# NVIDIA/semantic-segmentation

Hardware: AMD Instinct MI355X
Metric: train images/sec HRNet-OCR-MScale 1024x1024 crop (higher is better)
Workload: dtype fp16; 1 GPU; train_cityscapes_sota: HRNet-OCR-MScale two-scale train step, RMI+BCE loss, crop 1024x1024, batch 1/GPU, SGD, synthetic Cityscapes-shaped batch, random init; global_batch=1, parallelism=dp1, hipgraph=True, optimizer=ssa_sgd_momentum_step, wgrad_side_stream_flush_at=256

## Files before the change

### semantic-segmentation_amd/csrc/conv_wgrad_head.hip

```cpp
#include "common.h"
#include "group.h"
#include "../../include/semseg_hip.h"

namespace {

typedef short s16x8_t __attribute__((ext_vector_type(8)));

__host__ __device__ constexpr int trs(int row_bytes) {
  int s = (row_bytes + 63) / 64;
  if ((s & 1) == 0) ++s;
  return s * 64;
}

__device__ __forceinline__ bf16x8_t tr8(const unsigned char* p, int stride_bytes) {
  const s16x4_t lo = ssa_tr16_b64(p);
  const s16x4_t hi = ssa_tr16_b64(p + 4 * stride_bytes);
  s16x8_t v = {lo[0], lo[1], lo[2], lo[3], hi[0], hi[1], hi[2], hi[3]};
  return __builtin_bit_cast(bf16x8_t, v);
}

struct WgradHeadArgs {
  const bf16_t* x; const bf16_t* dy; float* partial;
  int ldx, Cin, lddy, cout_pad, B, H, W, tiles_x, tiles_y, tiles_per_wg, ci_tiles, G, wgs_y;
};

__device__ __forceinline__ int xcd_order(int v, int n) {
  const int q = n >> 3, r = n & 7, x = v & 7, k = v >> 3;
  return (x < r ? x * (q + 1) : r * (q + 1) + (x - r) * q) + k;
}

template <int KS>
struct ConvWgradHead {
  typedef WgradHeadArgs Args;
  static constexpr int NT = 512;
  static __device__ __forceinline__ void run(const Args& a, const int bx_, const int by0_, const int ) {
  const int w_ = xcd_order(by0_ * a.G + bx_, a.G * a.wgs_y);
  const int bx = w_ / a.wgs_y, by_ = w_ - bx * a.wgs_y;
  const bf16_t* __restrict__ x = a.x;
  const bf16_t* __restrict__ dy = a.dy;
  float* __restrict__ partial = a.partial;
  const int ldx = a.ldx, Cin = a.Cin, lddy = a.lddy, cout_pad = a.cout_pad, B = a.B, H = a.H, W = a.W;
  const int tiles_x = a.tiles_x, tiles_y = a.tiles_y, tiles_per_wg = a.tiles_per_wg, ci_tiles = a.ci_tiles;
  constexpr int TW = 32, TH = 4, NT = KS == 3 ? 3 : 2;
  constexpr int CX = KS == 3 ? 128 : 256;
  constexpr int XW = KS == 3 ? TW + 2 : TW;
  constexpr int SX = trs(CX * 2), SD = trs(256);
  constexpr int X_BYTES = TH * XW * SX;
  constexpr int XP = CX / 8, DP = 16;
  constexpr int XN = TH * XW * XP, DN = TH * TW * DP;
  constexpr int XI = (XN + 511) / 512, DI = (DN + 511) / 512;
  SSA_DYN_LDS(unsigned char, smem);
  unsigned char* Xs = smem;
  unsigned char* Ds = smem + X_BYTES;

  const int tid = threadIdx.x, lane = tid & 63;
  const int wave = __builtin_amdgcn_readfirstlane(tid >> 6);
  const int wm = wave >> 2, wn = wave & 3;
  int by = by_;
  const int kh = KS == 3 ? by % 3 : 0;
  if (KS == 3) by /= 3;
  const int ci_t = by % ci_tiles, co_t = by / ci_tiles;
  const int co0 = co_t * 128, ci0 = ci_t * CX;
  const int taps = KS * KS, Kflat = taps * Cin;

  const int li = lane & 15, lj = li >> 2, lq = li & 3, lg = (lane >> 4) & 1, lh = lane >> 5;
  int b_off[NT];
#pragma unroll
  for (int j = 0; j < NT; ++j) {
    const int cblk = KS == 3 ? wn : 2 * wn + j;
    const int shift = KS == 3 ? j : 0;
    b_off[j] = shift * SX + (cblk * 32 + 16 * lg + 4 * lq) * 2;
  }
  const int a_col = (16 * lg + 4 * lq) * 2;

  f32x16_t acc[2][NT];
#pragma unroll
  for (int m = 0; m < 2; ++m)
#pragma unroll
    for (int j = 0; j < NT; ++j)
#pragma unroll
      for (int r = 0; r < 16; ++r) acc[m][j][r] = 0.f;

  const int total_tiles = B * tiles_x * tiles_y;
  const int t_begin = bx * tiles_per_wg;
  const int t_end = min(total_tiles, t_begin + tiles_per_wg);
  uint4 xv[XI], dv[DI];
  unsigned xmask = 0, dmask = 0;
  auto fetch = [&](int t) {
    int r_ = t;
    const int tx_i = r_ % tiles_x; r_ /= tiles_x;
    const int ty_i = r_ % tiles_y;
    const int b = r_ / tiles_y;
    const int x0 = tx_i * TW, y0 = ty_i * TH;
    const int yoff = KS == 3 ? kh - 1 : 0, xoff = KS == 3 ? -1 : 0;
    const bf16_t* xb = x + (long)b * H * W * ldx + ci0;
    const bf16_t* db = dy + (long)b * H * W * lddy + co0;
#pragma unroll
    for (int i = 0; i < XI; ++i) {
      const int piece = tid + i * 512;
      const int pix = piece / XP, cp = piece - pix * XP;
      const int hy = pix / XW, hx = pix - hy * XW;
      const int iy = y0 + hy + yoff, ix = x0 + hx + xoff;
      const bool ok = piece < XN && (unsigned)iy < (unsigned)H && (unsigned)ix < (unsigned)W && ci0 + cp * 8 < Cin;
      xv[i] = *reinterpret_cast<const uint4*>(ok ? xb + ((long)iy * W + ix) * ldx + cp * 8 : x);
      xmask = i == 0 ? (ok ? 1u : 0u) : (xmask | ((ok ? 1u : 0u) << i));
    }
#pragma unroll
    for (int i = 0; i < DI; ++i) {
      const int piece = tid + i * 512;
      const int pix = piece / DP, cp = piece - pix * DP;
      const int oy = y0 + pix / TW, ox = x0 + pix % TW;
      const bool ok = piece < DN && oy < H && ox < W && co0 + cp * 8 < cout_pad;
      dv[i] = *reinterpret_cast<const uint4*>(ok ? db + ((long)oy * W + ox) * lddy + cp * 8 : dy);
      dmask = i == 0 ? (ok ? 1u : 0u) : (dmask | ((ok ? 1u : 0u) << i));
    }
  };
  auto stage = [&]() {
#pragma unroll
    for (int i = 0; i < XI; ++i) {
      const int piece = tid + i * 512;
      if (piece < XN)
        *reinterpret_cast<uint4*>(Xs + (piece / XP) * SX + (piece % XP) * 16) = ((xmask >> i) & 1u) ? xv[i] : make_uint4(0, 0, 0, 0);
    }
#pragma unroll
    for (int i = 0; i < DI; ++i) {
      const int piece = tid + i * 512;
      if (piece < DN)
        *reinterpret_cast<uint4*>(Ds + (piece / DP) * SD + (piece % DP) * 16) = ((dmask >> i) & 1u) ? dv[i] : make_uint4(0, 0, 0, 0);
    }
  };

  if (t_begin < t_end) fetch(t_begin);
  for (int t = t_begin; t < t_end; ++t) {
    if (t > t_begin) __syncthreads();
    stage();
    __syncthreads();
    if (t + 1 < t_end) fetch(t + 1);
    bf16x8_t af[2][2], bfr[2][NT];
    auto rd = [&](int ks, int slot) {
      const int ty = ks >> 1, kp = (ks & 1) * 16 + 8 * lh + lj;
#pragma unroll
      for (int m = 0; m < 2; ++m) af[slot][m] = tr8(Ds + (ty * TW + kp) * SD + (wm * 2 + m) * 64 + a_col, SD);
#pragma unroll
      for (int j = 0; j < NT; ++j) bfr[slot][j] = tr8(Xs + (ty * XW + kp) * SX + b_off[j], SX);
    };
    rd(0, 0);
    __builtin_amdgcn_sched_group_barrier(0x100, 2 * (2 + NT), 0);
#pragma unroll
    for (int ks = 0; ks < 8; ++ks) {
      if (ks + 1 < 8) rd(ks + 1, (ks + 1) & 1);
#pragma unroll
      for (int m = 0; m < 2; ++m)
#pragma unroll
        for (int j = 0; j < NT; ++j)
          acc[m][j] = ssa_mfma32(af[ks & 1][m], bfr[ks & 1][j], acc[m][j]);
      if (ks + 1 < 8) __builtin_amdgcn_sched_group_barrier(0x100, 2 * (2 + NT), 0);
      __builtin_amdgcn_sched_group_barrier(0x008, 2 * NT, 0);
    }
  }

  float* out = partial + (long)bx * cout_pad * Kflat;
#pragma unroll
  for (int m = 0; m < 2; ++m)
#pragma unroll
    for (int j = 0; j < NT; ++j) {
      const int cblk = KS == 3 ? wn : 2 * wn + j;
      const int ci = ci0 + cblk * 32 + (lane & 31);
      const int tap = KS == 3 ? kh * 3 + j : 0;
      if (ci >= Cin) continue;
      const long kcol = (long)tap * Cin + ci;
#pragma unroll
      for (int r = 0; r < 16; ++r) {
        const int co = co0 + (wm * 2 + m) * 32 + (r & 3) + 8 * (r >> 2) + 4 * (lane >> 5);
        if (co < cout_pad) out[(long)co * Kflat + kcol] = acc[m][j][r];
      }
    }
  }
};

__device__ uint4 g_zero_piece;

struct ConvWgradHead3 {
  typedef WgradHeadArgs Args;
  static constexpr int NT = 512;
  static constexpr int TW = 32, TH = 4, XW = TW + 2, CX = 128;
  static constexpr int X_BYTES = TH * XW * 256, D_BYTES = TH * TW * 256, BUF_BYTES = X_BYTES + D_BYTES;
  static constexpr int XWI = X_BYTES / 1024;
  static constexpr int XI = (XWI + 7) / 8, DI = D_BYTES / 1024 / 8, NI = XI + DI;
  static_assert(NI == 9, "one DMA in front of the k loop and one behind each of its 8 steps");
  static constexpr size_t LDS = 2 * (size_t)BUF_BYTES + 1024;
  static __device__ __forceinline__ void run(const Args& a, const int bx_, const int by0_, const int ) {
  const int w_ = xcd_order(by0_ * a.G + bx_, a.G * a.wgs_y);
  const int bx = w_ / a.wgs_y;
  int by = w_ - bx * a.wgs_y;
  const bf16_t* __restrict__ x = a.x;
  const bf16_t* __restrict__ dy = a.dy;
  float* __restrict__ partial = a.partial;
  const int ldx = a.ldx, Cin = a.Cin, lddy = a.lddy, cout_pad = a.cout_pad, B = a.B, H = a.H, W = a.W;
  const int tiles_x = a.tiles_x, tiles_y = a.tiles_y, tiles_per_wg = a.tiles_per_wg, ci_tiles = a.ci_tiles;
  SSA_DYN_LDS(unsigned char, smem);
  unsigned char* dump = smem + 2 * BUF_BYTES;

  const int tid = threadIdx.x, lane = tid & 63;
  const int wave = __builtin_amdgcn_readfirstlane(tid >> 6);
  const int wm = wave >> 2, wn = wave & 3;
  const int kh = by % 3; by /= 3;
  const int ci_t = by % ci_tiles, co_t = by / ci_tiles;
  const int co0 = co_t * 128, ci0 = ci_t * CX;
  const int Kflat = 9 * Cin;

  int rel[NI], yx[NI];
#pragma unroll
  for (int i = 0; i < NI; ++i) {
    const bool isx = i < XI;
    const int wi = (isx ? i : i - XI) * 8 + wave;
    const int piece = wi * 64 + lane;
    const int p = piece >> 4, q = (piece & 15) ^ ((p & 3) << 2);
    const int r = isx ? p / XW : p >> 5, c = isx ? p - r * XW : p & 31;
    const bool real = isx ? (wi < XWI && ci0 + q * 8 < Cin) : (co0 + q * 8 < cout_pad);
    rel[i] = (r * W + c) * (isx ? ldx : lddy) + q * 8;
    yx[i] = real ? ((r << 8) | c) : 0xffff;
  }
  int f_tx, f_ty, f_b;
  const int total_tiles = B * tiles_x * tiles_y;
  const int t_begin = bx * tiles_per_wg;
  const int t_end = min(total_tiles, t_begin + tiles_per_wg);
  {
    f_tx = t_begin % tiles_x;
    const int r_ = t_begin / tiles_x;
    f_ty = r_ % tiles_y;
    f_b = r_ / tiles_y;
  }
  const bf16_t* zero_src = reinterpret_cast<const bf16_t*>(&g_zero_piece);
#ifndef SSA_EMU
  asm volatile("" : "+v"(zero_src));
#endif
  auto dma = [&](int i, int buf) {
    const int x0 = f_tx * TW, y0 = f_ty * TH;
    const bool isx = i < XI;
    const int wi = (isx ? i : i - XI) * 8 + wave;
    const int oy = isx ? y0 + kh - 1 : y0, ox = isx ? x0 - 1 : x0;
    const bf16_t* base = (isx ? x + ci0 : dy + co0) + ((long)f_b * H * W + (long)oy * W + ox) * (isx ? ldx : lddy);
    const int iy = oy + (yx[i] >> 8), ix = ox + (yx[i] & 255);
    const bool ok = yx[i] != 0xffff && (unsigned)iy < (unsigned)H && (unsigned)ix < (unsigned)W;
    const bf16_t* src = ok ? base + rel[i] : zero_src;
    unsigned char* Xb = smem + buf * BUF_BYTES;
    unsigned char* dst = isx ? (wi < XWI ? Xb + wi * 1024 : dump) : Xb + X_BYTES + wi * 1024;
    ssa_glds16_untracked(src, dst);
  };
  auto next_tile = [&]() {
    if (++f_tx == tiles_x) {
      f_tx = 0;
      if (++f_ty == tiles_y) { f_ty = 0; ++f_b; }
    }
  };

  const int li = lane & 15, lj = li >> 2, lq = li & 3, lg = (lane >> 4) & 1, lh = lane >> 5;
  const int lrow = (8 * lh + lj) * 256 + lg * 32 + lq * 8;
  int a_base[2], b_base[4];
#pragma unroll
  for (int m = 0; m < 2; ++m) a_base[m] = X_BYTES + lrow + (((wm * 2 + m) ^ lj) << 6);
#pragma unroll
  for (int r = 0; r < 4; ++r) b_base[r] = lrow + ((wn ^ ((lj + r) & 3)) << 6);

  f32x16_t acc[2][3];
#pragma unroll
  for (int m = 0; m < 2; ++m)
#pragma unroll
    for (int j = 0; j < 3; ++j)
#pragma unroll
      for (int r = 0; r < 16; ++r) acc[m][j][r] = 0.f;

  if (t_begin < t_end) {
#pragma unroll
    for (int i = 0; i < NI; ++i) dma(i, 0);
    next_tile();
    ssa_wait_vm_barrier<0, 0>();
  }
  for (int t = t_begin; t < t_end; ++t) {
    const int buf = (t - t_begin) & 1;
    const bool more = t + 1 < t_end;
    if (more) dma(0, buf ^ 1);
    const unsigned char* Tb = smem + buf * BUF_BYTES;
    bf16x8_t af[2][2], bfr[2][3];
    auto rd = [&](int ks, int slot) {
      const int ty = ks >> 1, kp = (ks & 1) * 16;
#pragma unroll
      for (int m = 0; m < 2; ++m) af[slot][m] = tr8(Tb + a_base[m] + (ty * TW + kp) * 256, 256);
#pragma unroll
      for (int j = 0; j < 3; ++j) bfr[slot][j] = tr8(Tb + b_base[(2 * ty + j) & 3] + (ty * XW + kp + j) * 256, 256);
    };
    rd(0, 0);
    __builtin_amdgcn_sched_group_barrier(0x100, 10, 0);
#pragma unroll
    for (int ks = 0; ks < 8; ++ks) {
      if (ks + 1 < 8) rd(ks + 1, (ks + 1) & 1);
#pragma unroll
      for (int m = 0; m < 2; ++m)
#pragma unroll
        for (int j = 0; j < 3; ++j)
          acc[m][j] = ssa_mfma32(af[ks & 1][m], bfr[ks & 1][j], acc[m][j]);
      if (more) dma(ks + 1, buf ^ 1);
      if (ks + 1 < 8) __builtin_amdgcn_sched_group_barrier(0x100, 10, 0);
      __builtin_amdgcn_sched_group_barrier(0x008, 6, 0);
      __builtin_amdgcn_sched_group_barrier(0x020, 1, 0);
    }
    if (more) next_tile();
    ssa_wait_vm_barrier<0, 0>();
  }

  float* out = partial + (long)bx * cout_pad * Kflat;
#pragma unroll
  for (int m = 0; m < 2; ++m)
#pragma unroll
    for (int j = 0; j < 3; ++j) {
      const int ci = ci0 + wn * 32 + (lane & 31);
      if (ci >= Cin) continue;
      const long kcol = (long)(kh * 3 + j) * Cin + ci;
#pragma unroll
      for (int r = 0; r < 16; ++r) {
        const int co = co0 + (wm * 2 + m) * 32 + (r & 3) + 8 * (r >> 2) + 4 * (lane >> 5);
        if (co < cout_pad) out[(long)co * Kflat + kcol] = acc[m][j][r];
      }
    }
  }
};

bool head_shape_ok(const ssa_conv_desc* d, int cout_pad) {
  if (!d || d->KH != d->KW || (d->KH != 3 && d->KH != 1)) return false;
  if (d->stride != 1 || d->dil != 1 || d->pad != d->KH / 2 || d->transposed) return false;
  if (d->Ho != d->H || d->Wo != d->W || d->ldx % 8 || d->Cin % 8 || cout_pad % 8) return false;
  return d->Cin >= 128 && cout_pad >= 64 && d->W >= 32 && (long)d->B * d->H * d->W >= 16384;
}

struct HeadPlan { int co_tiles, ci_tiles, wgs_y, G, tpw; long per_split; };

HeadPlan head_plan(const ssa_conv_desc& d, int cout_pad) {
  HeadPlan p;
  const int cx = d.KH == 3 ? 128 : 256;
  p.co_tiles = (cout_pad + 127) / 128;
  p.ci_tiles = (d.Cin + cx - 1) / cx;
  p.wgs_y = p.co_tiles * p.ci_tiles * (d.KH == 3 ? 3 : 1);
  const long tiles = (long)d.B * ((d.W + 31) / 32) * ((d.H + 3) / 4);
  long g = 256 / p.wgs_y;
  if (g < 1) g = 1;
  if (g > tiles) g = tiles;
  p.tpw = (int)((tiles + g - 1) / g);
  p.G = (int)((tiles + p.tpw - 1) / p.tpw);
  p.per_split = (long)cout_pad * d.KH * d.KW * d.Cin * sizeof(float);
  return p;
}

void fill_args(WgradHeadArgs& a, const ssa_conv_desc& d, const HeadPlan& p, const void* x, const void* dy, int lddy,
               int cout_pad, float* partial) {
  a.x = (const bf16_t*)x; a.dy = (const bf16_t*)dy; a.partial = partial;
  a.ldx = d.ldx; a.Cin = d.Cin; a.lddy = lddy; a.cout_pad = cout_pad; a.B = d.B; a.H = d.H; a.W = d.W;
  a.tiles_x = (d.W + 31) / 32; a.tiles_y = (d.H + 3) / 4; a.tiles_per_wg = p.tpw; a.ci_tiles = p.ci_tiles;
  a.G = p.G; a.wgs_y = p.wgs_y;
}

template <int KS>
int launch_head(const ssa_conv_desc& d, const HeadPlan& p, const void* x, const void* dy, int lddy,
                int cout_pad, float* partial, hipStream_t s) {
  constexpr int XW = KS == 3 ? 34 : 32, CX = KS == 3 ? 128 : 256;
  constexpr size_t lds = (size_t)4 * XW * trs(CX * 2) + (size_t)128 * trs(256);
  static_assert(lds <= 160 * 1024, "does not fit in LDS");
  WgradHeadArgs a;
  fill_args(a, d, p, x, dy, lddy, cout_pad, partial);
  return ssa::submit<ConvWgradHead<KS>>(a, p.G, p.wgs_y, lds, s);
}

}

extern "C" {

int ssa_conv2d_wgrad_head_plan(const ssa_conv_desc* d, int cout_pad, int* nsplit, size_t* ws_bytes) {
  if (!nsplit || !ws_bytes || !head_shape_ok(d, cout_pad)) return SSA_EUNSUPPORTED;
  const HeadPlan p = head_plan(*d, cout_pad);
  *nsplit = p.G;
  *ws_bytes = (size_t)p.G * p.per_split;
  return SSA_OK;
}

int ssa_conv2d_wgrad_head(const ssa_conv_desc* dp, const void* x, const void* dy, int lddy, int cout_pad,
                          int nsplit, float* partial, void* stream) {
  if (!dp || !x || !dy || !partial) return SSA_EINVAL;
  if (!head_shape_ok(dp, cout_pad) || lddy % 8) return SSA_EUNSUPPORTED;
  if ((reinterpret_cast<uintptr_t>(x) | reinterpret_cast<uintptr_t>(dy)) & 15u) return SSA_EINVAL;
  const HeadPlan p = head_plan(*dp, cout_pad);
  if (nsplit != p.G) return SSA_EINVAL;
  if (dp->KH == 3) {
    WgradHeadArgs a;
    fill_args(a, *dp, p, x, dy, lddy, cout_pad, partial);
    return ssa::submit<ConvWgradHead3>(a, p.G, p.wgs_y, ConvWgradHead3::LDS, (hipStream_t)stream);
  }
  return launch_head<1>(*dp, p, x, dy, lddy, cout_pad, partial, (hipStream_t)stream);
}

}
```

Before: 52.37 images/s.

## Restructure head wgrad kernels: async DMA 1x1 path, all-tap 3x3 tiles

The 1x1 head weight-gradient kernel now treats pixels as a flat 64-pixel K dimension. Operands are loaded with double-buffered global-to-LDS DMA and XOR-swizzled LDS, replacing register staging. A selectable 256-wide co tile (MB=8) is chosen by a byte-traffic heuristic, trading fewer passes over x against larger split partials. The 3x3 kernel no longer splits work across kh into separate workgroups: each workgroup loads a 6-row halo with 64 input channels and computes all 9 taps, split 5/4 across two wave groups, which cuts redundant dy reads but raises per-workgroup accumulator pressure.

```diff
diff --git a/semantic-segmentation_amd/csrc/conv_wgrad_head.hip b/semantic-segmentation_amd/csrc/conv_wgrad_head.hip
--- a/semantic-segmentation_amd/csrc/conv_wgrad_head.hip
+++ b/semantic-segmentation_amd/csrc/conv_wgrad_head.hip
@@ -1,16 +1,11 @@
 #include "common.h"
 #include "group.h"
 #include "../../include/semseg_hip.h"
+#include <type_traits>
 
 namespace {
 
 typedef short s16x8_t __attribute__((ext_vector_type(8)));
-
-__host__ __device__ constexpr int trs(int row_bytes) {
-  int s = (row_bytes + 63) / 64;
-  if ((s & 1) == 0) ++s;
-  return s * 64;
-}
 
 __device__ __forceinline__ bf16x8_t tr8(const unsigned char* p, int stride_bytes) {
   const s16x4_t lo = ssa_tr16_b64(p);
@@ -29,170 +24,151 @@
   return (x < r ? x * (q + 1) : r * (q + 1) + (x - r) * q) + k;
 }
 
-template <int KS>
+__device__ uint4 g_zero_piece;
+
+__device__ __forceinline__ const bf16_t* zero_piece() {
+  const bf16_t* z = reinterpret_cast<const bf16_t*>(&g_zero_piece);
+#ifndef SSA_EMU
+  asm volatile("" : "+v"(z));
+#endif
+  return z;
+}
+
+template <int MB>
 struct ConvWgradHead {
   typedef WgradHeadArgs Args;
   static constexpr int NT = 512;
+  static constexpr int KP = 64, CX = 256;
+  static constexpr int SXP = CX * 2, SDP = MB * 64;
+  static constexpr int X_BYTES = KP * SXP, D_BYTES = KP * SDP, BUF_BYTES = X_BYTES + D_BYTES;
+  static constexpr int XI = X_BYTES / 1024 / 8, DI = D_BYTES / 1024 / 8, NI = XI + DI;
+  static constexpr int WM = MB / 2, WN = 8 / WM, NB = 8 / WN;
+  static constexpr size_t LDS = 2 * (size_t)BUF_BYTES;
+  static_assert((MB == 4 || MB == 8) && LDS <= 160 * 1024, "geometry");
   static __device__ __forceinline__ void run(const Args& a, const int bx_, const int by0_, const int ) {
   const int w_ = xcd_order(by0_ * a.G + bx_, a.G * a.wgs_y);
-  const int bx = w_ / a.wgs_y, by_ = w_ - bx * a.wgs_y;
+  const int bx = w_ / a.wgs_y, by = w_ - bx * a.wgs_y;
   const bf16_t* __restrict__ x = a.x;
   const bf16_t* __restrict__ dy = a.dy;
   float* __restrict__ partial = a.partial;
-  const int ldx = a.ldx, Cin = a.Cin, lddy = a.lddy, cout_pad = a.cout_pad, B = a.B, H = a.H, W = a.W;
-  const int tiles_x = a.tiles_x, tiles_y = a.tiles_y, tiles_per_wg = a.tiles_per_wg, ci_tiles = a.ci_tiles;
-  constexpr int TW = 32, TH = 4, NT = KS == 3 ? 3 : 2;
-  constexpr int CX = KS == 3 ? 128 : 256;
-  constexpr int XW = KS == 3 ? TW + 2 : TW;
-  constexpr int SX = trs(CX * 2), SD = trs(256);
-  constexpr int X_BYTES = TH * XW * SX;
-  constexpr int XP = CX / 8, DP = 16;
-  constexpr int XN = TH * XW * XP, DN = TH * TW * DP;
-  constexpr int XI = (XN + 511) / 512, DI = (DN + 511) / 512;
+  const int ldx = a.ldx, Cin = a.Cin, lddy = a.lddy, cout_pad = a.cout_pad;
   SSA_DYN_LDS(unsigned char, smem);
-  unsigned char* Xs = smem;
-  unsigned char* Ds = smem + X_BYTES;
 
   const int tid = threadIdx.x, lane = tid & 63;
   const int wave = __builtin_amdgcn_readfirstlane(tid >> 6);
-  const int wm = wave >> 2, wn = wave & 3;
-  int by = by_;
-  const int kh = KS == 3 ? by % 3 : 0;
-  if (KS == 3) by /= 3;
-  const int ci_t = by % ci_tiles, co_t = by / ci_tiles;
-  const int co0 = co_t * 128, ci0 = ci_t * CX;
-  const int taps = KS * KS, Kflat = taps * Cin;
+  const int wm = wave / WN, wn = wave % WN;
+  const int ci_t = by % a.ci_tiles, co_t = by / a.ci_tiles;
+  const int co0 = co_t * (MB * 32), ci0 = ci_t * CX;
+  const int Kflat = Cin;
+
+  int pk[NI];
+#pragma unroll
+  for (int i = 0; i < NI; ++i) {
+    const bool isx = i < XI;
+    const int slot = ((isx ? i : i - XI) * 8 + wave) * 64 + lane;
+    const int pp = isx ? SXP / 16 : SDP / 16;
+    const int p = slot / pp, q = (slot % pp) ^ ((p & 3) << 2);
+    const bool real = isx ? ci0 + q * 8 < Cin : co0 + q * 8 < cout_pad;
+    pk[i] = real ? ((p << 8) | q) : -1;
+  }
+  const int pixels = a.B * a.H * a.W;
+  const int total = (pixels + KP - 1) / KP;
+  const int s_begin = bx * a.tiles_per_wg;
+  const int s_end = min(total, s_begin + a.tiles_per_wg);
+  const bf16_t* zero_src = zero_piece();
+  auto dma = [&](int i, int s, int buf) {
+    const bool isx = i < XI;
+    const int wi = (isx ? i : i - XI) * 8 + wave;
+    const int pix = s * KP + (pk[i] >> 8);
+    const bool ok = pk[i] >= 0 && pix < pixels;
+    const bf16_t* src = ok ? (isx ? x + ci0 + (long)pix * ldx : dy + co0 + (long)pix * lddy) + (pk[i] & 255) * 8 : zero_src;
+    ssa_glds16_untracked(src, smem + buf * BUF_BYTES + (isx ? 0 : X_BYTES) + wi * 1024);
+  };
 
   const int li = lane & 15, lj = li >> 2, lq = li & 3, lg = (lane >> 4) & 1, lh = lane >> 5;
-  int b_off[NT];
-#pragma unroll
-  for (int j = 0; j < NT; ++j) {
-    const int cblk = KS == 3 ? wn : 2 * wn + j;
-    const int shift = KS == 3 ? j : 0;
-    b_off[j] = shift * SX + (cblk * 32 + 16 * lg + 4 * lq) * 2;
-  }
-  const int a_col = (16 * lg + 4 * lq) * 2;
-
-  f32x16_t acc[2][NT];
+  const int lcol = lg * 32 + lq * 8;
+  int a_base[2], b_base[NB];
+#pragma unroll
+  for (int m = 0; m < 2; ++m) a_base[m] = X_BYTES + (8 * lh + lj) * SDP + lcol + (((wm * 2 + m) ^ lj) << 6);
+#pragma unroll
+  for (int j = 0; j < NB; ++j) b_base[j] = (8 * lh + lj) * SXP + lcol + (((wn * NB + j) ^ lj) << 6);
+
+  f32x16_t acc[2][NB];
 #pragma unroll
   for (int m = 0; m < 2; ++m)
 #pragma unroll
-    for (int j = 0; j < NT; ++j)
+    for (int j = 0; j < NB; ++j)
 #pragma unroll
       for (int r = 0; r < 16; ++r) acc[m][j][r] = 0.f;
 
-  const int total_tiles = B * tiles_x * tiles_y;
-  const int t_begin = bx * tiles_per_wg;
-  const int t_end = min(total_tiles, t_begin + tiles_per_wg);
-  uint4 xv[XI], dv[DI];
-  unsigned xmask = 0, dmask = 0;
-  auto fetch = [&](int t) {
-    int r_ = t;
-    const int tx_i = r_ % tiles_x; r_ /= tiles_x;
-    const int ty_i = r_ % tiles_y;
-    const int b = r_ / tiles_y;
-    const int x0 = tx_i * TW, y0 = ty_i * TH;
-    const int yoff = KS == 3 ? kh - 1 : 0, xoff = KS == 3 ? -1 : 0;
-    const bf16_t* xb = x + (long)b * H * W * ldx + ci0;
-    const bf16_t* db = dy + (long)b * H * W * lddy + co0;
-#pragma unroll
-    for (int i = 0; i < XI; ++i) {
-      const int piece = tid + i * 512;
-      const int pix = piece / XP, cp = piece - pix * XP;
-      const int hy = pix / XW, hx = pix - hy * XW;
-      const int iy = y0 + hy + yoff, ix = x0 + hx + xoff;
-      const bool ok = piece < XN && (unsigned)iy < (unsigned)H && (unsigned)ix < (unsigned)W && ci0 + cp * 8 < Cin;
-      xv[i] = *reinterpret_cast<const uint4*>(ok ? xb + ((long)iy * W + ix) * ldx + cp * 8 : x);
-      xmask = i == 0 ? (ok ? 1u : 0u) : (xmask | ((ok ? 1u : 0u) << i));
-    }
-#pragma unroll
-    for (int i = 0; i < DI; ++i) {
-      const int piece = tid + i * 512;
-      const int pix = piece / DP, cp = piece - pix * DP;
-      const int oy = y0 + pix / TW, ox = x0 + pix % TW;
-      const bool ok = piece < DN && oy < H && ox < W && co0 + cp * 8 < cout_pad;
-      dv[i] = *reinterpret_cast<const uint4*>(ok ? db + ((long)oy * W + ox) * lddy + cp * 8 : dy);
-      dmask = i == 0 ? (ok ? 1u : 0u) : (dmask | ((ok ? 1u : 0u) << i));
-    }
-  };
-  auto stage = [&]() {
-#pragma unroll
-    for (int i = 0; i < XI; ++i) {
-      const int piece = tid + i * 512;
-      if (piece < XN)
-        *reinterpret_cast<uint4*>(Xs + (piece / XP) * SX + (piece % XP) * 16) = ((xmask >> i) & 1u) ? xv[i] : make_uint4(0, 0, 0, 0);
-    }
-#pragma unroll
-    for (int i = 0; i < DI; ++i) {
-      const int piece = tid + i * 512;
-      if (piece < DN)
-        *reinterpret_cast<uint4*>(Ds + (piece / DP) * SD + (piece % DP) * 16) = ((dmask >> i) & 1u) ? dv[i] : make_uint4(0, 0, 0, 0);
-    }
-  };
-
-  if (t_begin < t_end) fetch(t_begin);
-  for (int t = t_begin; t < t_end; ++t) {
-    if (t > t_begin) __syncthreads();
-    stage();
-    __syncthreads();
-    if (t + 1 < t_end) fetch(t + 1);
-    bf16x8_t af[2][2], bfr[2][NT];
+  if (s_begin < s_end) {
+#pragma unroll
+    for (int i = 0; i < NI; ++i) dma(i, s_begin, 0);
+    ssa_wait_vm_barrier<0, 0>();
+  }
+  for (int s = s_begin; s < s_end; ++s) {
+    const int buf = (s - s_begin) & 1;
+    const bool more = s + 1 < s_end;
+    const unsigned char* Tb = smem + buf * BUF_BYTES;
+    bf16x8_t af[2][2], bfr[2][NB];
     auto rd = [&](int ks, int slot) {
-      const int ty = ks >> 1, kp = (ks & 1) * 16 + 8 * lh + lj;
-#pragma unroll
-      for (int m = 0; m < 2; ++m) af[slot][m] = tr8(Ds + (ty * TW + kp) * SD + (wm * 2 + m) * 64 + a_col, SD);
-#pragma unroll
-      for (int j = 0; j < NT; ++j) bfr[slot][j] = tr8(Xs + (ty * XW + kp) * SX + b_off[j], SX);
+#pragma unroll
+      for (int m = 0; m < 2; ++m) af[slot][m] = tr8(Tb + a_base[m] + ks * 16 * SDP, SDP);
+#pragma unroll
+      for (int j = 0; j < NB; ++j) bfr[slot][j] = tr8(Tb + b_base[j] + ks * 16 * SXP, SXP);
     };
     rd(0, 0);
-    __builtin_amdgcn_sched_group_barrier(0x100, 2 * (2 + NT), 0);
-#pragma unroll
-    for (int ks = 0; ks < 8; ++ks) {
-      if (ks + 1 < 8) rd(ks + 1, (ks + 1) & 1);
+    __builtin_amdgcn_sched_group_barrier(0x100, 2 * (2 + NB), 0);
+#pragma unroll
+    for (int ks = 0; ks < 4; ++ks) {
+      if (ks + 1 < 4) rd(ks + 1, (ks + 1) & 1);
 #pragma unroll
       for (int m = 0; m < 2; ++m)
 #pragma unroll
-        for (int j = 0; j < NT; ++j)
+        for (int j = 0; j < NB; ++j)
           acc[m][j] = ssa_mfma32(af[ks & 1][m], bfr[ks & 1][j], acc[m][j]);
-      if (ks + 1 < 8) __builtin_amdgcn_sched_group_barrier(0x100, 2 * (2 + NT), 0);
-      __builtin_amdgcn_sched_group_barrier(0x008, 2 * NT, 0);
-    }
+      if (more) {
+#pragma unroll
+        for (int i = ks * NI / 4; i < (ks + 1) * NI / 4; ++i) dma(i, s + 1, buf ^ 1);
+      }
+      if (ks + 1 < 4) __builtin_amdgcn_sched_group_barrier(0x100, 2 * (2 + NB), 0);
+      __builtin_amdgcn_sched_group_barrier(0x008, 2 * NB, 0);
+      __builtin_amdgcn_sched_group_barrier(0x020, (NI + 3) / 4, 0);
+    }
+    ssa_wait_vm_barrier<0, 0>();
   }
 
   float* out = partial + (long)bx * cout_pad * Kflat;
 #pragma unroll
   for (int m = 0; m < 2; ++m)
 #pragma unroll
-    for (int j = 0; j < NT; ++j) {
-      const int cblk = KS == 3 ? wn : 2 * wn + j;
-      const int ci = ci0 + cblk * 32 + (lane & 31);
-      const int tap = KS == 3 ? kh * 3 + j : 0;
+    for (int j = 0; j < NB; ++j) {
+      const int ci = ci0 + (wn * NB + j) * 32 + (lane & 31);
       if (ci >= Cin) continue;
-      const long kcol = (long)tap * Cin + ci;
 #pragma unroll
       for (int r = 0; r < 16; ++r) {
         const int co = co0 + (wm * 2 + m) * 32 + (r & 3) + 8 * (r >> 2) + 4 * (lane >> 5);
-        if (co < cout_pad) out[(long)co * Kflat + kcol] = acc[m][j][r];
+        if (co < cout_pad) out[(long)co * Kflat + ci] = acc[m][j][r];
       }
     }
   }
 };
-
-__device__ uint4 g_zero_piece;
 
 struct ConvWgradHead3 {
   typedef WgradHeadArgs Args;
   static constexpr int NT = 512;
-  static constexpr int TW = 32, TH = 4, XW = TW + 2, CX = 128;
-  static constexpr int X_BYTES = TH * XW * 256, D_BYTES = TH * TW * 256, BUF_BYTES = X_BYTES + D_BYTES;
-  static constexpr int XWI = X_BYTES / 1024;
+  static constexpr int TW = 32, TH = 4, XW = TW + 2, XH = TH + 2, CX = 64;
+  static constexpr int SXP = CX * 2, SDP = 256;
+  static constexpr int XN = XH * XW * (SXP / 16);
+  static constexpr int XWI = (XN + 63) / 64;
+  static constexpr int X_BYTES = XWI * 1024, D_BYTES = TH * TW * SDP, BUF_BYTES = X_BYTES + D_BYTES;
   static constexpr int XI = (XWI + 7) / 8, DI = D_BYTES / 1024 / 8, NI = XI + DI;
-  static_assert(NI == 9, "one DMA in front of the k loop and one behind each of its 8 steps");
+  static_assert(NI == 8, "one DMA behind each of the 8 k-steps");
   static constexpr size_t LDS = 2 * (size_t)BUF_BYTES + 1024;
+  static_assert(LDS <= 160 * 1024, "does not fit in LDS");
   static __device__ __forceinline__ void run(const Args& a, const int bx_, const int by0_, const int ) {
   const int w_ = xcd_order(by0_ * a.G + bx_, a.G * a.wgs_y);
-  const int bx = w_ / a.wgs_y;
-  int by = w_ - bx * a.wgs_y;
+  const int bx = w_ / a.wgs_y, by = w_ - bx * a.wgs_y;
   const bf16_t* __restrict__ x = a.x;
   const bf16_t* __restrict__ dy = a.dy;
   float* __restrict__ partial = a.partial;
@@ -203,23 +179,21 @@
 
   const int tid = threadIdx.x, lane = tid & 63;
   const int wave = __builtin_amdgcn_readfirstlane(tid >> 6);
-  const int wm = wave >> 2, wn = wave & 3;
-  const int kh = by % 3; by /= 3;
+  const int tg = wave >> 2, mp = (wave >> 1) & 1, nb = wave & 1;
   const int ci_t = by % ci_tiles, co_t = by / ci_tiles;
   const int co0 = co_t * 128, ci0 = ci_t * CX;
   const int Kflat = 9 * Cin;
 
-  int rel[NI], yx[NI];
+  int pk[NI];
 #pragma unroll
   for (int i = 0; i < NI; ++i) {
     const bool isx = i < XI;
-    const int wi = (isx ? i : i - XI) * 8 + wave;
-    const int piece = wi * 64 + lane;
-    const int p = piece >> 4, q = (piece & 15) ^ ((p & 3) << 2);
+    const int slot = ((isx ? i : i - XI) * 8 + wave) * 64 + lane;
+    const int p = isx ? slot >> 3 : slot >> 4;
+    const int q = isx ? (slot & 7) ^ (((p >> 1) & 1) << 2) : (slot & 15) ^ ((p & 3) << 2);
     const int r = isx ? p / XW : p >> 5, c = isx ? p - r * XW : p & 31;
-    const bool real = isx ? (wi < XWI && ci0 + q * 8 < Cin) : (co0 + q * 8 < cout_pad);
-    rel[i] = (r * W + c) * (isx ? ldx : lddy) + q * 8;
-    yx[i] = real ? ((r << 8) | c) : 0xffff;
+    const bool real = isx ? (slot < XN && ci0 + q * 8 < Cin) : (co0 + q * 8 < cout_pad);
+    pk[i] = real ? ((r << 12) | (c << 4) | q) : -1;
   }
   int f_tx, f_ty, f_b;
   const int total_tiles = B * tiles_x * tiles_y;
@@ -231,19 +205,15 @@
     f_ty = r_ % tiles_y;
     f_b = r_ / tiles_y;
   }
-  const bf16_t* zero_src = reinterpret_cast<const bf16_t*>(&g_zero_piece);
-#ifndef SSA_EMU
-  asm volatile("" : "+v"(zero_src));
-#endif
+  const bf16_t* zero_src = zero_piece();
   auto dma = [&](int i, int buf) {
-    const int x0 = f_tx * TW, y0 = f_ty * TH;
     const bool isx = i < XI;
     const int wi = (isx ? i : i - XI) * 8 + wave;
-    const int oy = isx ? y0 + kh - 1 : y0, ox = isx ? x0 - 1 : x0;
-    const bf16_t* base = (isx ? x + ci0 : dy + co0) + ((long)f_b * H * W + (long)oy * W + ox) * (isx ? ldx : lddy);
-    const int iy = oy + (yx[i] >> 8), ix = ox + (yx[i] & 255);
-    const bool ok = yx[i] != 0xffff && (unsigned)iy < (unsigned)H && (unsigned)ix < (unsigned)W;
-    const bf16_t* src = ok ? base + rel[i] : zero_src;
+    const int oy = f_ty * TH - (isx ? 1 : 0), ox = f_tx * TW - (isx ? 1 : 0);
+    const int iy = oy + (pk[i] >> 12), ix = ox + ((pk[i] >> 4) & 255);
+    const bool ok = pk[i] >= 0 && (unsigned)iy < (unsigned)H && (unsigned)ix < (unsigned)W;
+    const bf16_t* img = (isx ? x + ci0 : dy + co0) + (long)f_b * H * W * (isx ? ldx : lddy);
+    const bf16_t* src = ok ? img + ((long)iy * W + ix) * (isx ? ldx : lddy) + (pk[i] & 15) * 8 : zero_src;
     unsigned char* Xb = smem + buf * BUF_BYTES;
     unsigned char* dst = isx ? (wi < XWI ? Xb + wi * 1024 : dump) : Xb + X_BYTES + wi * 1024;
     ssa_glds16_untracked(src, dst);
@@ -256,73 +226,80 @@
   };
 
   const int li = lane & 15, lj = li >> 2, lq = li & 3, lg = (lane >> 4) & 1, lh = lane >> 5;
-  const int lrow = (8 * lh + lj) * 256 + lg * 32 + lq * 8;
-  int a_base[2], b_base[4];
-#pragma unroll
-  for (int m = 0; m < 2; ++m) a_base[m] = X_BYTES + lrow + (((wm * 2 + m) ^ lj) << 6);
-#pragma unroll
-  for (int r = 0; r < 4; ++r) b_base[r] = lrow + ((wn ^ ((lj + r) & 3)) << 6);
-
-  f32x16_t acc[2][3];
-#pragma unroll
-  for (int m = 0; m < 2; ++m)
-#pragma unroll
-    for (int j = 0; j < 3; ++j)
-#pragma unroll
-      for (int r = 0; r < 16; ++r) acc[m][j][r] = 0.f;
-
-  if (t_begin < t_end) {
-#pragma unroll
-    for (int i = 0; i < NI; ++i) dma(i, 0);
-    next_tile();
-    ssa_wait_vm_barrier<0, 0>();
-  }
-  for (int t = t_begin; t < t_end; ++t) {
-    const int buf = (t - t_begin) & 1;
-    const bool more = t + 1 < t_end;
-    if (more) dma(0, buf ^ 1);
-    const unsigned char* Tb = smem + buf * BUF_BYTES;
-    bf16x8_t af[2][2], bfr[2][3];
-    auto rd = [&](int ks, int slot) {
-      const int ty = ks >> 1, kp = (ks & 1) * 16;
-#pragma unroll
-      for (int m = 0; m < 2; ++m) af[slot][m] = tr8(Tb + a_base[m] + (ty * TW + kp) * 256, 256);
-#pragma unroll
-      for (int j = 0; j < 3; ++j) bfr[slot][j] = tr8(Tb + b_base[(2 * ty + j) & 3] + (ty * XW + kp + j) * 256, 256);
-    };
-    rd(0, 0);
-    __builtin_amdgcn_sched_group_barrier(0x100, 10, 0);
-#pragma unroll
-    for (int ks = 0; ks < 8; ++ks) {
-      if (ks + 1 < 8) rd(ks + 1, (ks + 1) & 1);
-#pragma unroll
-      for (int m = 0; m < 2; ++m)
-#pragma unroll
-        for (int j = 0; j < 3; ++j)
-          acc[m][j] = ssa_mfma32(af[ks & 1][m], bfr[ks & 1][j], acc[m][j]);
-      if (more) dma(ks + 1, buf ^ 1);
-      if (ks + 1 < 8) __builtin_amdgcn_sched_group_barrier(0x100, 10, 0);
-      __builtin_amdgcn_sched_group_barrier(0x008, 6, 0);
-      __builtin_amdgcn_sched_group_barrier(0x020, 1, 0);
-    }
-    if (more) next_tile();
-    ssa_wait_vm_barrier<0, 0>();
-  }
-
-  float* out = partial + (long)bx * cout_pad * Kflat;
-#pragma unroll
-  for (int m = 0; m < 2; ++m)
-#pragma unroll
-    for (int j = 0; j < 3; ++j) {
-      const int ci = ci0 + wn * 32 + (lane & 31);
-      if (ci >= Cin) continue;
-      const long kcol = (long)(kh * 3 + j) * Cin + ci;
-#pragma unroll
-      for (int r = 0; r < 16; ++r) {
-        const int co = co0 + (wm * 2 + m) * 32 + (r & 3) + 8 * (r >> 2) + 4 * (lane >> 5);
-        if (co < cout_pad) out[(long)co * Kflat + kcol] = acc[m][j][r];
+  const int lcol = lg * 32 + lq * 8;
+  int a_base[2], b_base[3];
+#pragma unroll
+  for (int m = 0; m < 2; ++m) a_base[m] = X_BYTES + (8 * lh + lj) * SDP + lcol + (((mp * 2 + m) ^ lj) << 6);
+#pragma unroll
+  for (int kw = 0; kw < 3; ++kw) b_base[kw] = (8 * lh + lj) * SXP + lcol + ((nb ^ (((kw + lj) >> 1) & 1)) << 6);
+
+  auto body = [&](auto tg_c) {
+    constexpr int T0 = decltype(tg_c)::value == 0 ? 0 : 5, NTAP = decltype(tg_c)::value == 0 ? 5 : 4;
+    f32x16_t acc[2][NTAP];
+#pragma unroll
+    for (int m = 0; m < 2; ++m)
+#pragma unroll
+      for (int j = 0; j < NTAP; ++j)
+#pragma unroll
+        for (int r = 0; r < 16; ++r) acc[m][j][r] = 0.f;
+
+    if (t_begin < t_end) {
+#pragma unroll
+      for (int i = 0; i < NI; ++i) dma(i, 0);
+      next_tile();
+      ssa_wait_vm_barrier<0, 0>();
+    }
+    for (int t = t_begin; t < t_end; ++t) {
+      const int buf = (t - t_begin) & 1;
+      const bool more = t + 1 < t_end;
+      const unsigned char* Tb = smem + buf * BUF_BYTES;
+      bf16x8_t af[2][2], bfr[2][NTAP];
+      auto rd = [&](int ks, int slot) {
+        const int ty = ks >> 1, kp = (ks & 1) * 16;
+#pragma unroll
+        for (int m = 0; m < 2; ++m) af[slot][m] = tr8(Tb + a_base[m] + (ty * TW + kp) * SDP, SDP);
+#pragma unroll
+        for (int j = 0; j < NTAP; ++j) {
+          const int kh = (T0 + j) / 3, kw = (T0 + j) % 3, row = ty + kh;
+          bfr[slot][j] = tr8(Tb + (b_base[kw] ^ ((row & 1) << 6)) + (row * XW + kp + kw) * SXP, SXP);
+        }
+      };
+      rd(0, 0);
+      __builtin_amdgcn_sched_group_barrier(0x100, 2 * (2 + NTAP), 0);
+#pragma unroll
+      for (int ks = 0; ks < 8; ++ks) {
+        if (ks + 1 < 8) rd(ks + 1, (ks + 1) & 1);
+#pragma unroll
+        for (int j = 0; j < NTAP; ++j)
+#pragma unroll
+          for (int m = 0; m < 2; ++m)
+            acc[m][j] = ssa_mfma32(af[ks & 1][m], bfr[ks & 1][j], acc[m][j]);
+        if (more) dma(ks, buf ^ 1);
+        if (ks + 1 < 8) __builtin_amdgcn_sched_group_barrier(0x100, 2 * (2 + NTAP), 0);
+        __builtin_amdgcn_sched_group_barrier(0x008, 2 * NTAP, 0);
+        __builtin_amdgcn_sched_group_barrier(0x020, 1, 0);
       }
-    }
+      if (more) next_tile();
+      ssa_wait_vm_barrier<0, 0>();
+    }
+
+    float* out = partial + (long)bx * cout_pad * Kflat;
+    const int ci = ci0 + nb * 32 + (lane & 31);
+    if (ci >= Cin) return;
+#pragma unroll
+    for (int m = 0; m < 2; ++m)
+#pragma unroll
+      for (int j = 0; j < NTAP; ++j) {
+        const long kcol = (long)(T0 + j) * Cin + ci;
+#pragma unroll
+        for (int r = 0; r < 16; ++r) {
+          const int co = co0 + (mp * 2 + m) * 32 + (r & 3) + 8 * (r >> 2) + 4 * (lane >> 5);
+          if (co < cout_pad) out[(long)co * Kflat + kcol] = acc[m][j][r];
+        }
+      }
+  };
+  if (tg == 0) body(std::integral_constant<int, 0>());
+  else body(std::integral_constant<int, 1>());
   }
 };
 
@@ -333,15 +310,17 @@
   return d->Cin >= 128 && cout_pad >= 64 && d->W >= 32 && (long)d->B * d->H * d->W >= 16384;
 }
 
-struct HeadPlan { int co_tiles, ci_tiles, wgs_y, G, tpw; long per_split; };
-
-HeadPlan head_plan(const ssa_conv_desc& d, int cout_pad) {
+struct HeadPlan { int mb, co_tiles, ci_tiles, wgs_y, G, tpw; long per_split; };
+
+HeadPlan head_plan_mb(const ssa_conv_desc& d, int cout_pad, int mb) {
   HeadPlan p;
-  const int cx = d.KH == 3 ? 128 : 256;
-  p.co_tiles = (cout_pad + 127) / 128;
+  const int cx = d.KH == 3 ? 64 : 256;
+  p.mb = mb;
+  p.co_tiles = (cout_pad + mb * 32 - 1) / (mb * 32);
   p.ci_tiles = (d.Cin + cx - 1) / cx;
-  p.wgs_y = p.co_tiles * p.ci_tiles * (d.KH == 3 ? 3 : 1);
-  const long tiles = (long)d.B * ((d.W + 31) / 32) * ((d.H + 3) / 4);
+  p.wgs_y = p.co_tiles * p.ci_tiles;
+  const long pixels = (long)d.B * d.H * d.W;
+  const long tiles = d.KH == 3 ? (long)d.B * ((d.W + 31) / 32) * ((d.H + 3) / 4) : (pixels + 63) / 64;
   long g = 256 / p.wgs_y;
   if (g < 1) g = 1;
   if (g > tiles) g = tiles;
@@ -351,23 +330,23 @@
   return p;
 }
 
+HeadPlan head_plan(const ssa_conv_desc& d, int cout_pad) {
+  const HeadPlan lo = head_plan_mb(d, cout_pad, 4);
+  if (d.KH == 3 || d.cfg == 1) return lo;
+  const HeadPlan hi = head_plan_mb(d, cout_pad, 8);
+  if (d.cfg == 2) return hi;
+  const double x_bytes = 2.0 * d.B * d.H * d.W * d.Cin;
+  const double saved = x_bytes * (lo.co_tiles - hi.co_tiles);
+  const double added = (double)hi.G * hi.per_split - (double)lo.G * lo.per_split;
+  return saved > 2.0 * added ? hi : lo;
+}
+
 void fill_args(WgradHeadArgs& a, const ssa_conv_desc& d, const HeadPlan& p, const void* x, const void* dy, int lddy,
                int cout_pad, float* partial) {
   a.x = (const bf16_t*)x; a.dy = (const bf16_t*)dy; a.partial = partial;
   a.ldx = d.ldx; a.Cin = d.Cin; a.lddy = lddy; a.cout_pad = cout_pad; a.B = d.B; a.H = d.H; a.W = d.W;
   a.tiles_x = (d.W + 31) / 32; a.tiles_y = (d.H + 3) / 4; a.tiles_per_wg = p.tpw; a.ci_tiles = p.ci_tiles;
   a.G = p.G; a.wgs_y = p.wgs_y;
-}
-
-template <int KS>
-int launch_head(const ssa_conv_desc& d, const HeadPlan& p, const void* x, const void* dy, int lddy,
-                int cout_pad, float* partial, hipStream_t s) {
-  constexpr int XW = KS == 3 ? 34 : 32, CX = KS == 3 ? 128 : 256;
-  constexpr size_t lds = (size_t)4 * XW * trs(CX * 2) + (size_t)128 * trs(256);
-  static_assert(lds <= 160 * 1024, "does not fit in LDS");
-  WgradHeadArgs a;
-  fill_args(a, d, p, x, dy, lddy, cout_pad, partial);
-  return ssa::submit<ConvWgradHead<KS>>(a, p.G, p.wgs_y, lds, s);
 }
 
 }
@@ -389,12 +368,12 @@
   if ((reinterpret_cast<uintptr_t>(x) | reinterpret_cast<uintptr_t>(dy)) & 15u) return SSA_EINVAL;
   const HeadPlan p = head_plan(*dp, cout_pad);
   if (nsplit != p.G) return SSA_EINVAL;
-  if (dp->KH == 3) {
-    WgradHeadArgs a;
-    fill_args(a, *dp, p, x, dy, lddy, cout_pad, partial);
-    return ssa::submit<ConvWgradHead3>(a, p.G, p.wgs_y, ConvWgradHead3::LDS, (hipStream_t)stream);
-  }
-  return launch_head<1>(*dp, p, x, dy, lddy, cout_pad, partial, (hipStream_t)stream);
-}
-
-}
+  WgradHeadArgs a;
+  fill_args(a, *dp, p, x, dy, lddy, cout_pad, partial);
+  hipStream_t s = (hipStream_t)stream;
+  if (dp->KH == 3) return ssa::submit<ConvWgradHead3>(a, p.G, p.wgs_y, ConvWgradHead3::LDS, s);
+  if (p.mb == 8) return ssa::submit<ConvWgradHead<8>>(a, p.G, p.wgs_y, ConvWgradHead<8>::LDS, s);
+  return ssa::submit<ConvWgradHead<4>>(a, p.G, p.wgs_y, ConvWgradHead<4>::LDS, s);
+}
+
+}
```

Result: no change. 52.59 images/s (median of 6 runs) (+0.4%).
